# johncai117/Meta-Fine-Tuning

Hardware: AMD Instinct MI355X
Metric: episodes/sec at 5-way N-shot (ResNet10+GNN) per GPU and 1/2/4/8-GPU node (higher is better)
Workload: dtype f32

## Files before the change

### meta-fine-tuning_amd/csrc/conv_igemm.hip

```cpp
#include "mft_common.h"
#include "mft_hip_testing.h"

int mft_stem_conv_dispatch(const float* in, const float* w, float* out, int n_img, int H, int W, int w_ld,
                           hipStream_t s);
int mft_skinny_fwd_dispatch(const float* in, int ldi, const float* w, float* out, int ldo, int n_img, int H, int W,
                            int Cin, int Cout, int KH, int KW, int stride, int pad, int imgs_per_group,
                            long long w_group_stride, hipStream_t s);
void mft_skinny_set_dgrad_slices(int n);
void mft_skinny_set_tap(int v);
void mft_skinny_set_x3(int v);
void mft_skinny_set_nw(int v);
void mft_bn_small_set_rows(int rows);
void mft_bn_fwd_small_set_rows(int rows);
void mft_skinny_set_lines(int v);
int mft_skinny_dgrad_dispatch(const float* dy, int ldy, const float* w, float* dx, int ldx, int n_img, int H, int W,
                              int Cin, int Cout, int KH, int KW, int stride, int pad, int imgs_per_group,
                              long long w_group_stride, hipStream_t s);

namespace {

struct ConvArgs {
    const float* in;
    const float* w;
    const float* bias;
// ... 1197 lines not shown
    else if (tile >= 9100) mft_skinny_set_nw(tile - 9100);
    else if (tile >= 9000) g_wgrad_pol = tile - 9000;
    else if (tile >= 8000) mft_skinny_set_x3(tile - 8000);
    else if (tile >= 7000) mft_skinny_set_tap(tile - 7000);
    else if (tile >= 6000) mft_skinny_set_dgrad_slices(tile - 6000);
    else if (tile >= 5000) g_wgrad_early = tile - 5000;
    else if (tile >= 4000) g_wgrad_min_lds_kb = tile - 4000;
    else if (tile >= 3000) g_skinny = tile - 3000;
    else if (tile >= 2100) g_stem_wgrad_strips = tile - 2100;
    else if (tile >= 2000) g_stem_fast = tile - 2000;
    else if (tile >= 1000) g_wgrad_tile = tile - 1000;
    else g_conv_tile = tile;
    return 0;
}

extern "C" int mft_debug_set_x3_tile(int t);

extern "C" void mft_wgrad_fwd_set_exact(int on);
extern "C" int mft_debug_reset(void) {
    mft_wgrad_fwd_set_exact(0);
    mft_wgrad_fwd_set_xcd(1);
    g_dgrad_parity = 1; g_wgrad_trim = 1; g_wgrad_rows = 1; g_wgrad_tile = 64; g_conv_tile = 0; g_wgrad_pol = 7; g_wgrad_early = 1; g_wgrad_min_lds_kb = 0; g_skinny = 1; g_stem_fast = 1; g_stem_wgrad_strips = 1;
    mft_skinny_set_lines(1); mft_skinny_set_nw(0); mft_skinny_set_x3(1); mft_skinny_set_tap(1); mft_skinny_set_dgrad_slices(1);
    mft_debug_set_x3_tile(0); mft_debug_set_x3_tile(10); mft_debug_set_x3_tile(21); mft_debug_set_x3_tile(31); mft_debug_set_x3_tile(41);
    mft_bn_small_set_rows(512); mft_bn_fwd_small_set_rows(512);
    mft_debug_set_x3_tile(60); mft_debug_set_x3_tile(70); mft_debug_set_x3_tile(80); mft_debug_set_x3_tile(91); mft_debug_set_x3_tile(100); mft_debug_set_x3_tile(200);
    return 0;
}

static int dgrad_impl(const float* dy, int ldy, const float* w, float* dx, int ldx, int n_img, int H,
                      int W, int Cin, int Cout, int KH, int KW, int stride, int pad,
                      int imgs_per_group, long long w_group_stride, float* ws, void* stream) {
    if (Cout % 32 != 0 || Cin % 4 != 0 || ldy % 4 != 0 || stride < 1) return MFT_EINVAL;
    if (imgs_per_group <= 0) imgs_per_group = n_img;
    if (n_img % imgs_per_group != 0) return MFT_EINVAL;
    const int groups = n_img / imgs_per_group;
    if (g_skinny && groups > 1 && w_group_stride != 0 && ws == nullptr) {
        const int rc = mft_skinny_dgrad_dispatch(dy, ldy, w, dx, ldx, n_img, H, W, Cin, Cout, KH, KW, stride, pad,
                                                 imgs_per_group, w_group_stride, (hipStream_t)stream);
        if (rc != MFT_EINVAL) return rc;
    }
    ConvArgs a;
    a.in = dy; a.w = w; a.bias = nullptr; a.out = dx;
    a.ldi = ldy; a.ldo = ldx;
    a.H = (H + 2 * pad - KH) / stride + 1;
    a.W = (W + 2 * pad - KW) / stride + 1;
    a.Cin = Cout; a.KH = KH; a.KW = KW;
// ... 181 lines not shown
```

### meta-fine-tuning_amd/csrc/conv_x3.hip

```cpp
#include "mft_common.h"
#include "bn_fold.h"

namespace {

typedef __bf16 bf16x8 __attribute__((ext_vector_type(8)));
typedef __bf16 bf16x2 __attribute__((ext_vector_type(2)));
typedef _Float16 f16x8 __attribute__((ext_vector_type(8)));
typedef _Float16 f16x4 __attribute__((ext_vector_type(4)));
typedef float f32x2 __attribute__((ext_vector_type(2)));
typedef unsigned u32x2 __attribute__((ext_vector_type(2)));
typedef unsigned u32x4 __attribute__((ext_vector_type(4)));

struct X3Args {
    const float* in;
    const unsigned short* w3;
    long long plane;
    float* out;
    int ldi, ldo;
    int H, W, Cin, OH, OW, Cout, KH, KW, stride, pad;
    int Kpad;
    int M;
    int tiles_n;
    unsigned in_bytes, w_bytes;
    int xcd_swizzle;
// ... 22 lines not shown
    r[0] = x[0] - __builtin_bit_cast(float, p1[0] << 16);
    r[1] = x[1] - __builtin_bit_cast(float, p1[0] & 0xffff0000u);
    r[2] = x[2] - __builtin_bit_cast(float, p1[1] << 16);
    r[3] = x[3] - __builtin_bit_cast(float, p1[1] & 0xffff0000u);
    p2[0] = pk_bf16(r[0], r[1]);
    p2[1] = pk_bf16(r[2], r[3]);
    r[0] -= __builtin_bit_cast(float, p2[0] << 16);
    r[1] -= __builtin_bit_cast(float, p2[0] & 0xffff0000u);
    r[2] -= __builtin_bit_cast(float, p2[1] << 16);
    r[3] -= __builtin_bit_cast(float, p2[1] & 0xffff0000u);
    p3[0] = pk_bf16(r[0], r[1]);
    p3[1] = pk_bf16(r[2], r[3]);
}

__device__ __forceinline__ void split4_h2(const f32x4 x, u32x2& p1, u32x2& p2) {
    const f16x4 hi = __builtin_convertvector(x, f16x4);
    const f32x4 r = (x - __builtin_convertvector(hi, f32x4)) * 2048.f;
    const f16x4 lo = __builtin_convertvector(r, f16x4);
    p1 = __builtin_bit_cast(u32x2, hi);
    p2 = __builtin_bit_cast(u32x2, lo);
}
constexpr float X3_H2_LO_SCALE = 1.0f / 2048.f;

template <int BM, int BN, bool AP, bool DB, int HOIST = 0, int DBG = 0, bool XS = false, int NP = 3>
__global__ __launch_bounds__(256) __attribute__((amdgpu_waves_per_eu(NP == 2 ? 3 : 1))) void conv_x3_kernel(X3Args p) {
    static_assert(NP == 3 || (NP == 2 && !AP && !DB && HOIST == 0 && DBG == 0 && !XS), "f16x2: the plain single-buffer form only");
    constexpr int NACC = NP == 3 ? 1 : 2;
    constexpr int TM = BM / 64;
    constexpr int TN = BN / 64;
    constexpr int PA = AP ? BM / 64 : BM / 32;
    constexpr int PB = BN / 64;
    constexpr int RS = XS ? 32 : X3_RS;
    constexpr int A_PLANE = BM * RS;
    constexpr int B_PLANE = BN * RS;
    auto lo = [](int row, int c) -> int {
        if constexpr (XS) return row * 32 + ((((c >> 3) ^ (row >> 2)) & 3) << 3) + (c & 7);
        else return row * X3_RS + c;
    };
    extern __shared__ __attribute__((aligned(16))) unsigned short smem[];
    unsigned short* As = smem;
    unsigned short* Bs = smem + NP * A_PLANE;
    constexpr int BUF = NP * (A_PLANE + B_PLANE);

    const int tid = threadIdx.x;
    const int lane = tid & 63, wave = tid >> 6;
    const int wm = wave >> 1, wn = wave & 1;
    const int r = lane & 31, h = lane >> 5;
    const bool g_swz = !XS && p.row_swz != 0;
    int tile_id = blockIdx.x;
    if (p.xcd_swizzle) {
        const int nwg = gridDim.x, q = nwg >> 3, rmd = nwg & 7;
        const int xcd = tile_id & 7, slot = tile_id >> 3;
        tile_id = xcd * q + (xcd < rmd ? xcd : rmd) + slot;
    }
    const int nt = tile_id % p.tiles_n;
    const int mt = tile_id / p.tiles_n;
    const int m0 = mt * BM, n0 = nt * BN;

    const int g_id = AP ? tid >> 4 : tid >> 5;
    const int g_rr = AP ? (tid >> 2) & 3 : (tid >> 3) & 3;
    const int lrow = g_swz ? g_rr * 4 + (g_id & 3) + 16 * (g_id >> 2) : (AP ? tid >> 2 : tid >> 3);
    const int c4 = AP ? (tid & 3) * 8 : (tid & 7) * 4;
    constexpr int RPP = AP ? 64 : 32;
    constexpr int ESZ = AP ? 2 : 4;
    const int ohw = p.OH * p.OW;
// ... 1 lines not shown
                                         : __builtin_amdgcn_make_buffer_rsrc((void*)p.in, 0, p.in_bytes, 0x00020000);
    const __amdgpu_buffer_rsrc_t rB = __builtin_amdgcn_make_buffer_rsrc((void*)p.w3, 0, p.w_bytes, 0x00020000);
    int a_off[PA];
    int a_ih0[PA], a_iw0[PA];
    bool a_ok[PA];
#pragma unroll
    for (int j = 0; j < PA; ++j) {
        const int m = m0 + lrow + RPP * j;
        a_ok[j] = m < p.M;
        const int mm = a_ok[j] ? m : 0;
        const int img = mm / ohw;
        const int rem = mm - img * ohw;
        const int oh = rem / p.OW, ow = rem - oh * p.OW;
        a_ih0[j] = oh * p.stride - p.pad;
        a_iw0[j] = ow * p.stride - p.pad;
        a_off[j] = (((img * p.H + a_ih0[j]) * p.W + a_iw0[j]) * p.ldi + c4) * ESZ;
    }
    const int bseg = tid & 3;
    const int brow = g_swz ? ((tid >> 2) & 3) * 4 + ((tid >> 4) & 3) + 16 * (tid >> 6) : tid >> 2;
    int b_off[PB];
#pragma unroll
    for (int j = 0; j < PB; ++j) b_off[j] = ((n0 + brow + 64 * j) * p.Kpad + bseg * 8) * 2;
    const int plane_bytes = (int)(p.plane * 2);

    f32x16 accs[NACC][TM][TN];
#pragma unroll
    for (int q = 0; q < NACC; ++q)
#pragma unroll
        for (int i = 0; i < TM; ++i)
#pragma unroll
            for (int j = 0; j < TN; ++j)
#pragma unroll
                for (int e = 0; e < 16; ++e) accs[q][i][j][e] = 0.f;
    auto& acc = accs[0];
    auto val = [&](int i, int j, int e) -> float {
        if constexpr (NP == 3) return accs[0][i][j][e];
        else return __builtin_fmaf(accs[NACC - 1][i][j][e], X3_H2_LO_SCALE, accs[0][i][j][e]);
    };

    struct Stage {
        f32x4 ra[AP ? 1 : PA];
        u32x4 ra3[AP ? PA : 1][3];
        u32x4 rb[PB][NP];
    };
    Stage st0;
    const int nk = p.Kpad / 32;

    int t_kt = 0, t_ci0 = 0, t_kh = 0, t_kw = 0;
    auto load_tile = [&](int kt, Stage& S) {
        const int k0 = kt * 32;
        while (t_kt < kt) {
            ++t_kt;
            t_ci0 += 32;
            if (t_ci0 == p.Cin) { t_ci0 = 0; if (++t_kw == p.KW) { t_kw = 0; ++t_kh; } }
        }
        const int ci0 = t_ci0, kh = t_kh, kw = t_kw;
        const int tap_off = ((kh * p.W + kw) * p.ldi + ci0) * ESZ;
#pragma unroll
        for (int j = 0; j < PA; ++j) {
            const bool ok = a_ok[j] && (unsigned)(a_ih0[j] + kh) < (unsigned)p.H && (unsigned)(a_iw0[j] + kw) < (unsigned)p.W;
            const unsigned voff = ok ? (unsigned)(a_off[j] + tap_off) : 0x80000000u;
            if constexpr (AP) {
#pragma unroll
                for (int pl = 0; pl < 3; ++pl)
                    S.ra3[j][pl] = __builtin_amdgcn_raw_buffer_load_b128(rA, voff, pl * (int)p.in_plane_bytes, 0);
            } else {
                S.ra[j] = __builtin_bit_cast(f32x4, __builtin_amdgcn_raw_buffer_load_b128(rA, voff, 0, 0));
            }
        }
#pragma unroll
        for (int j = 0; j < PB; ++j)
#pragma unroll
            for (int pl = 0; pl < NP; ++pl)
                S.rb[j][pl] = __builtin_amdgcn_raw_buffer_load_b128(rB, b_off[j] + pl * plane_bytes, k0 * 2, 0);
    };
    auto store_tile = [&](const Stage& S, int buf) {
        unsigned short* As = smem + buf * BUF;
        unsigned short* Bs = As + NP * A_PLANE;
#pragma unroll
        for (int j = 0; j < PA; ++j) {
            const int off = lo(lrow + RPP * j, c4);
            if constexpr (NP == 2) {
                u32x2 p1, p2;
                split4_h2(S.ra[j], p1, p2);
                *(u32x2*)(As + off) = p1;
                *(u32x2*)(As + A_PLANE + off) = p2;
            } else if constexpr (AP) {
#pragma unroll
                for (int pl = 0; pl < 3; ++pl) *(u32x4*)(As + pl * A_PLANE + off) = S.ra3[j][pl];
            } else {
                u32x2 p1, p2, p3;
                if constexpr (DBG & 1) {
                    const u32x4 raw = __builtin_bit_cast(u32x4, S.ra[j]);
                    p1[0] = raw[0]; p1[1] = raw[1]; p2[0] = raw[2]; p2[1] = raw[3]; p3 = p1;
                } else {
                    split4(S.ra[j], p1, p2, p3);
                }
                *(u32x2*)(As + off) = p1;
                *(u32x2*)(As + A_PLANE + off) = p2;
                *(u32x2*)(As + 2 * A_PLANE + off) = p3;
            }
        }
#pragma unroll
        for (int j = 0; j < PB; ++j)
#pragma unroll
            for (int pl = 0; pl < NP; ++pl)
                *(u32x4*)(Bs + pl * B_PLANE + lo(brow + 64 * j, bseg * 8)) = S.rb[j][pl];
    };

    auto compute = [&](int buf) {
        const unsigned short* As = smem + buf * BUF;
        const unsigned short* Bs = As + NP * A_PLANE;
        if constexpr (NP == 2) {
#pragma unroll
            for (int kk = 0; kk < 2; ++kk) {
                f16x8 a[TM][2], b[TN][2];
#pragma unroll
                for (int i = 0; i < TM; ++i)
#pragma unroll
                    for (int pl = 0; pl < 2; ++pl)
                        a[i][pl] = *(const f16x8*)(As + pl * A_PLANE + lo(wm * (BM / 2) + i * 32 + r, kk * 16 + h * 8));
#pragma unroll
                for (int j = 0; j < TN; ++j)
#pragma unroll
                    for (int pl = 0; pl < 2; ++pl)
                        b[j][pl] = *(const f16x8*)(Bs + pl * B_PLANE + lo(wn * (BN / 2) + j * 32 + r, kk * 16 + h * 8));
                constexpr int TA[3] = {0, 1, 0};
                constexpr int TB[3] = {1, 0, 0};
                constexpr int TQ[3] = {1, 1, 0};
#pragma unroll
                for (int t = 0; t < 3; ++t)
#pragma unroll
                    for (int i = 0; i < TM; ++i)
#pragma unroll
                        for (int j = 0; j < TN; ++j)
                            accs[TQ[t] ? NACC - 1 : 0][i][j] =
                                __builtin_amdgcn_mfma_f32_32x32x16_f16(a[i][TA[t]], b[j][TB[t]], accs[TQ[t] ? NACC - 1 : 0][i][j], 0, 0, 0);
            }
            return;
        }
        if constexpr (HOIST == 0) {
#pragma unroll
            for (int kk = 0; kk < 2; ++kk) {
                bf16x8 a[TM][3], b[TN][3];
#pragma unroll
                for (int i = 0; i < TM; ++i)
#pragma unroll
                    for (int pl = 0; pl < 3; ++pl)
                        a[i][pl] = *(const bf16x8*)(As + pl * A_PLANE + lo(wm * (BM / 2) + i * 32 + r, kk * 16 + h * 8));
// ... 79 lines not shown
            rd(1);
            mm(0);
            for (int q = 0; q < 6 * TM * TN; ++q) {
                __builtin_amdgcn_sched_group_barrier(0x8, 1, 0);
                __builtin_amdgcn_sched_group_barrier(0x100, (3 * (TM + TN) + 6 * TM * TN - 1) / (6 * TM * TN), 0);
            }
            __builtin_amdgcn_sched_barrier(0);
            mm(1);
            __builtin_amdgcn_sched_barrier(0);
        }
    };
    if constexpr (DB) {
        load_tile(0, st0);
        store_tile(st0, 0);
        __syncthreads();
        load_tile(nk > 1 ? 1 : 0, st0);
        for (int kt = 0; kt + 1 < nk; ++kt) {
            compute(kt & 1);
            store_tile(st0, (kt + 1) & 1);
            load_tile(kt + 2 < nk ? kt + 2 : nk - 1, st0);
            __syncthreads();
        }
        compute((nk - 1) & 1);
    } else {
        load_tile(0, st0);
        store_tile(st0, 0);
        __syncthreads();
        for (int kt = 0; kt < nk; ++kt) {
            if constexpr (!(DBG & 4)) { if (kt + 1 < nk) load_tile(kt + 1, st0); }
            if constexpr (!(DBG & 16)) compute(0);
            if constexpr (!(DBG & 32)) __syncthreads();
            if constexpr (!(DBG & 8)) { if (kt + 1 < nk) store_tile(st0, 0); }
            if constexpr (!(DBG & 32)) __syncthreads();
        }
    }

#pragma unroll
    for (int i = 0; i < TM; ++i)
#pragma unroll
        for (int j = 0; j < TN; ++j) {
            const int n = n0 + wn * (BN / 2) + j * 32 + r;
#pragma unroll
            for (int e = 0; e < 16; ++e) {
                const int row = (e & 3) + 8 * (e >> 2) + 4 * h;
                const int m = m0 + wm * (BM / 2) + i * 32 + row;
                if (m < p.M) p.out[(long long)m * p.ldo + n] = val(i, j, e);
// ... 25 lines not shown
                o[0] = a1; o[1] = a2; o[2] = b1; o[3] = b2;
            }
        }
        __syncthreads();
        if (wm == 0 && h == 0) {
#pragma unroll
            for (int j = 0; j < TN; ++j) {
                const float* o0 = sred + ((((0 * 2 + wn) * TN + j) * 32 + r) << 2);
                const float* o1 = sred + ((((1 * 2 + wn) * TN + j) * 32 + r) << 2);
                const int n = n0 + wn * (BN / 2) + j * 32 + r;
                float* w0 = p.stats_ws + (((long long)mt * 2 + 0) * p.Cout + n) * 2;
                float* w1 = p.stats_ws + (((long long)mt * 2 + 1) * p.Cout + n) * 2;
                w0[0] = o0[0] + o1[0]; w0[1] = o0[1] + o1[1];
                w1[0] = o0[2] + o1[2]; w1[1] = o0[3] + o1[3];
            }
        }
    }
}

#ifdef MFT_EXPERIMENTS
#include "../../tools/experiments/conv_x3_pingpong.inc"
#endif

template <int BM, int BN, bool BNIN, int NP = 3, bool BDB = true>
__device__ __forceinline__ void conv_x3_s1_body(const X3Args& p) {
    static_assert(NP == 3 || NP == 2, "3 bf16 pieces (six products) or 2 fp16 pieces (three products)");
    constexpr int NACC = NP == 3 ? 1 : 2;
    constexpr int TM = BM / 64, TN = BN / 64;
    constexpr int PA = BM / 32, PB = BN / 64;
    constexpr int RS = X3_RS;
    constexpr int B_PLANE = BN * RS;
    const int A_PLANE = p.s1_rows * RS;
    extern __shared__ __attribute__((aligned(16))) unsigned short smem[];
    constexpr int NBB = (NP == 2 && BDB) ? 2 : 1;
    unsigned short* As = smem;
    unsigned short* Bs = smem + NP * A_PLANE;
    float* bn_tab = reinterpret_cast<float*>(Bs + NBB * NP * B_PLANE);

    const int tid = threadIdx.x;
    const int lane = tid & 63, wave = tid >> 6;
    const int wm = wave >> 1, wn = wave & 1;
    const int r = lane & 31, h = lane >> 5;
    int tile_id = blockIdx.x;
    if (p.xcd_swizzle) {
        const int nwg = gridDim.x, q = nwg >> 3, rmd = nwg & 7;
        const int xcd = tile_id & 7, slot = tile_id >> 3;
        tile_id = xcd * q + (xcd < rmd ? xcd : rmd) + slot;
    }
    const int nt = tile_id % p.tiles_n;
    const int mt = tile_id / p.tiles_n;
    const int m0 = mt * BM, n0 = nt * BN;
    const int W = p.W, H = p.H;
    const int fr0 = m0 / W;
    const int g0 = BNIN ? m0 / p.rows_per_group : 0;
    const bool bn_two = BNIN && (m0 + (BM < p.M - m0 ? BM : p.M - m0) - 1) / p.rows_per_group > g0;
    if constexpr (BNIN) {
        char* stage = reinterpret_cast<char*>(smem);
// ... 26 lines not shown
        const int t = lrow + 32 * j, m = m0 + t;
        const int fr = m / W;
        a_ok[j] = m < p.M;
        a_oh[j] = fr - (fr / H) * H;
        a_off[j] = ((a_ok[j] ? m : 0) * p.ldi + c4) * 4;
        a_lds[j] = (t + 1) * RS + c4;
        a_tab[j] = BNIN ? ((a_ok[j] ? m / p.rows_per_group - g0 : 0) * 2 * p.Cin + c4) : 0;
    }
    const int hside = (tid >> 3) & 1;
    const int mh = hside ? m0 + BM : m0 - 1;
    const int frh = (mh > 0 ? mh : 0) / W;
    const bool h_ok = tid < 16 && (hside ? (mh < p.M && mh - frh * W != 0) : (m0 > 0 && m0 - fr0 * W != 0));
    const int h_oh = frh - (frh / H) * H;
    const int h_off = ((h_ok ? mh : 0) * p.ldi + c4) * 4;
    const int h_lds = (hside ? BM + 1 : 0) * RS + c4;
    const int h_tab = BNIN ? (((hside && h_ok) ? (m0 + BM - 1) / p.rows_per_group - g0 : 0) * 2 * p.Cin + c4) : 0;

    const int bseg = tid & 3;
    const int brow = p.row_swz ? ((tid >> 2) & 3) * 4 + ((tid >> 4) & 3) + 16 * (tid >> 6) : tid >> 2;
    int b_off[PB];
#pragma unroll
    for (int j = 0; j < PB; ++j) b_off[j] = ((n0 + brow + 64 * j) * p.Kpad + bseg * 8) * 2;
    const int plane_bytes = (int)(p.plane * 2);

    int fa[TM], fl[TM], fr_[TM];
    constexpr int Z0 = BM + 2;
#pragma unroll
    for (int i = 0; i < TM; ++i) {
        const int t = wm * (BM / 2) + i * 32 + r;
        const int ow = (m0 + t) - ((m0 + t) / W) * W;
        fa[i] = (t + 1) * RS;
        fl[i] = ow == 0 ? (Z0 + ((t - Z0) & 15)) * RS : fa[i] - RS;
        fr_[i] = ow == W - 1 ? (Z0 + ((t + 2 - Z0) & 15)) * RS : fa[i] + RS;
    }

    f32x16 acc[NACC][TM][TN];
#pragma unroll
    for (int q = 0; q < NACC; ++q)
#pragma unroll
        for (int i = 0; i < TM; ++i)
#pragma unroll
            for (int j = 0; j < TN; ++j)
#pragma unroll
                for (int e = 0; e < 16; ++e) acc[q][i][j][e] = 0.f;
    auto val = [&](int i, int j, int e) -> float {
        if constexpr (NP == 3) return acc[0][i][j][e];
// ... 7 lines not shown
    };
    Stage st;
    const int n_ci = p.Cin / 32;
    const int n_ms = 3 * n_ci;
    auto load_a = [&](int ms, Stage& S) {
        const int kh = ms / n_ci, ci0 = (ms - kh * n_ci) * 32;
        const int shift = ((kh - 1) * W * p.ldi + ci0) * 4;
#pragma unroll
        for (int j = 0; j < PA; ++j) {
            const bool ok = a_ok[j] && (unsigned)(a_oh[j] + kh - 1) < (unsigned)H;
            S.ra[j] = __builtin_bit_cast(f32x4, __builtin_amdgcn_raw_buffer_load_b128(rA, ok ? (unsigned)(a_off[j] + shift) : 0x80000000u, 0, 0));
        }
        const bool okh = h_ok && (unsigned)(h_oh + kh - 1) < (unsigned)H;
        S.rh = __builtin_bit_cast(f32x4, __builtin_amdgcn_raw_buffer_load_b128(rA, okh ? (unsigned)(h_off + shift) : 0x80000000u, 0, 0));
    };
    auto load_b = [&](int ms, int kw, Stage& S) {
        const int kh = ms / n_ci, ci0 = (ms - kh * n_ci) * 32;
        const int k0 = (kh * 3 + kw) * p.Cin + ci0;
#pragma unroll
        for (int j = 0; j < PB; ++j)
#pragma unroll
            for (int pl = 0; pl < NP; ++pl)
                S.rb[j][pl] = __builtin_amdgcn_raw_buffer_load_b128(rB, b_off[j] + pl * plane_bytes, k0 * 2, 0);
    };
    auto put_a = [&](const f32x4 v, int off) {
        if constexpr (NP == 3) {
            u32x2 p1, p2, p3;
            split4(v, p1, p2, p3);
            *(u32x2*)(As + off) = p1;
            *(u32x2*)(As + A_PLANE + off) = p2;
            *(u32x2*)(As + 2 * A_PLANE + off) = p3;
        } else {
            u32x2 p1, p2;
            split4_h2(v, p1, p2);
            *(u32x2*)(As + off) = p1;
            *(u32x2*)(As + A_PLANE + off) = p2;
        }
    };
    auto bn_relu = [&](const f32x4 v, const f32x4 sc, const f32x4 sh, bool ok) {
        f32x4 o = mft_bn_affine4(v, sc, sh);
#pragma unroll
        for (int e = 0; e < 4; ++e) o[e] = ok ? fmaxf(o[e], 0.f) : 0.f;
        return o;
    };
    auto store_a = [&](const Stage& S, int ms) {
        if constexpr (BNIN) {
// ... 42 lines not shown
#pragma unroll
                    for (int pl = 0; pl < 3; ++pl)
                        b[j][pl] = *(const bf16x8*)(Bc + pl * B_PLANE + (wn * (BN / 2) + j * 32 + r) * RS + kk * 16 + h * 8);
                constexpr int TA[6] = {2, 0, 1, 1, 0, 0};
                constexpr int TB[6] = {0, 2, 1, 0, 1, 0};
#pragma unroll
                for (int t = 0; t < 6; ++t)
#pragma unroll
                    for (int i = 0; i < TM; ++i)
#pragma unroll
                        for (int j = 0; j < TN; ++j)
                            acc[0][i][j] = __builtin_amdgcn_mfma_f32_32x32x16_bf16(a[i][TA[t]], b[j][TB[t]], acc[0][i][j], 0, 0, 0);
            } else {
                f16x8 a[TM][2], b[TN][2];
#pragma unroll
                for (int i = 0; i < TM; ++i)
#pragma unroll
                    for (int pl = 0; pl < 2; ++pl)
                        a[i][pl] = *(const f16x8*)(As + pl * A_PLANE + (kw == 0 ? fl[i] : (kw == 1 ? fa[i] : fr_[i])) + kk * 16 + h * 8);
#pragma unroll
                for (int j = 0; j < TN; ++j)
#pragma unroll
                    for (int pl = 0; pl < 2; ++pl)
                        b[j][pl] = *(const f16x8*)(Bc + pl * B_PLANE + (wn * (BN / 2) + j * 32 + r) * RS + kk * 16 + h * 8);
                constexpr int TA[3] = {0, 1, 0};
                constexpr int TB[3] = {1, 0, 0};
                constexpr int TQ[3] = {1, 1, 0};
#pragma unroll
                for (int t = 0; t < 3; ++t)
#pragma unroll
                    for (int i = 0; i < TM; ++i)
#pragma unroll
                        for (int j = 0; j < TN; ++j)
                            acc[TQ[t]][i][j] = __builtin_amdgcn_mfma_f32_32x32x16_f16(a[i][TA[t]], b[j][TB[t]], acc[TQ[t]][i][j], 0, 0, 0);
            }
        }
    };

    for (int i = tid; i < NP * A_PLANE / 8; i += 256) ((u32x4*)As)[i] = (u32x4){0u, 0u, 0u, 0u};
    load_a(0, st);
    load_b(0, 0, st);
    __syncthreads();
    store_a(st, 0);
    store_b(st);
    __syncthreads();
    if constexpr (NBB == 2) {
        int cur = 0;
        for (int ms = 0; ms < n_ms; ++ms) {
            const int msn = ms + 1 < n_ms ? ms + 1 : ms;
            load_b(ms, 1, st);
            compute(0, cur);
            store_b(st, cur ^ 1);
            __syncthreads();
            load_b(ms, 2, st);
            compute(1, cur ^ 1);
            store_b(st, cur);
            __syncthreads();
            load_a(msn, st);
            load_b(msn, 0, st);
            compute(2, cur);
            store_b(st, cur ^ 1);
            __syncthreads();
// ... 3 lines not shown
        }
    } else {
        for (int ms = 0; ms < n_ms; ++ms) {
            const int msn = ms + 1 < n_ms ? ms + 1 : ms;
            load_b(ms, 1, st);
            compute(0);
            __syncthreads();
            store_b(st);
            __syncthreads();
            load_b(ms, 2, st);
            compute(1);
            __syncthreads();
            store_b(st);
            __syncthreads();
            load_a(msn, st);
            load_b(msn, 0, st);
            compute(2);
            __syncthreads();
            store_a(st, msn);
            store_b(st);
            __syncthreads();
        }
    }

#pragma unroll
    for (int i = 0; i < TM; ++i)
#pragma unroll
        for (int j = 0; j < TN; ++j) {
            const int n = n0 + wn * (BN / 2) + j * 32 + r;
#pragma unroll
            for (int e = 0; e < 16; ++e) {
                const int row = (e & 3) + 8 * (e >> 2) + 4 * h;
                const int m = m0 + wm * (BM / 2) + i * 32 + row;
                if (m < p.M) p.out[(long long)m * p.ldo + n] = val(i, j, e);
            }
        }
    if (p.stats_ws != nullptr) {
        static_assert(TN == 1 || TN == 2, "stats epilogue");
        const int split = (m0 / p.rows_per_group + 1) * p.rows_per_group;
        float* sred = reinterpret_cast<float*>(smem);
        __syncthreads();
#pragma unroll
        for (int j = 0; j < TN; ++j) {
            float a1 = 0.f, a2 = 0.f, b1 = 0.f, b2 = 0.f;
#pragma unroll
            for (int i = 0; i < TM; ++i)
// ... 9 lines not shown
            a1 += __shfl_xor(a1, 32, 64); a2 += __shfl_xor(a2, 32, 64);
            b1 += __shfl_xor(b1, 32, 64); b2 += __shfl_xor(b2, 32, 64);
            if (h == 0) {
                float* o = sred + ((((wm * 2 + wn) * TN + j) * 32 + r) << 2);
                o[0] = a1; o[1] = a2; o[2] = b1; o[3] = b2;
            }
        }
        __syncthreads();
        if (wm == 0 && h == 0) {
#pragma unroll
            for (int j = 0; j < TN; ++j) {
                const float* o0 = sred + ((((0 * 2 + wn) * TN + j) * 32 + r) << 2);
                const float* o1 = sred + ((((1 * 2 + wn) * TN + j) * 32 + r) << 2);
                const int n = n0 + wn * (BN / 2) + j * 32 + r;
                float* w0 = p.stats_ws + (((long long)mt * 2 + 0) * p.Cout + n) * 2;
                float* w1 = p.stats_ws + (((long long)mt * 2 + 1) * p.Cout + n) * 2;
                w0[0] = o0[0] + o1[0]; w0[1] = o0[1] + o1[1];
                w1[0] = o0[2] + o1[2]; w1[1] = o0[3] + o1[3];
            }
        }
    }
}

template <int BM, int BN, int NP = 3, bool BDB = true>
__global__ __launch_bounds__(256) __attribute__((amdgpu_waves_per_eu(NP == 2 ? 3 : 1))) void conv_x3_s1_kernel(X3Args p) {
    conv_x3_s1_body<BM, BN, false, NP, BDB>(p);
}

template <int BM, int BN, int NP = 3, bool BDB = true>
__global__ __launch_bounds__(256) __attribute__((amdgpu_waves_per_eu(3, 3))) void conv_x3_s1_bnin_kernel(X3Args p) {
    conv_x3_s1_body<BM, BN, true, NP, BDB>(p);
}

__global__ void x3_stats_finalize_kernel(const float* __restrict__ ws, int C, int M, int R, int BM, float eps,
                                         float* __restrict__ mean, float* __restrict__ rstd) {
    const int c = blockIdx.x * blockDim.x + threadIdx.x;
    const int g = blockIdx.y;
    if (c >= C) return;
    float mu, rs;
    mft_x3_stats_merge(ws, C, c, g, M, R, BM, eps, mu, rs);
    mean[(long long)g * C + c] = mu;
    rstd[(long long)g * C + c] = rs;
}

__global__ __launch_bounds__(256) void split_bf16x3_kernel(const float* __restrict__ w, unsigned short* __restrict__ out,
                                                           long long n) {
    for (long long i = (long long)blockIdx.x * blockDim.x + threadIdx.x; i < n; i += (long long)gridDim.x * blockDim.x) {
        const float x = w[i];
        const unsigned q1 = pk_bf16(x, 0.f) & 0xffffu;
        const float r1 = x - __builtin_bit_cast(float, q1 << 16);
        const unsigned q2 = pk_bf16(r1, 0.f) & 0xffffu;
        const float r2 = r1 - __builtin_bit_cast(float, q2 << 16);
        const unsigned q3 = pk_bf16(r2, 0.f) & 0xffffu;
        out[i] = (unsigned short)q1;
// ... 26 lines not shown
        const float r2 = r1 - __builtin_bit_cast(float, q2 << 16);
        const unsigned q3 = pk_bf16(r2, 0.f) & 0xffffu;
        j.dst[l] = (unsigned short)q1;
        j.dst[j.n + l] = (unsigned short)q2;
        j.dst[2 * j.n + l] = (unsigned short)q3;
    }
}

__global__ __launch_bounds__(256) void split_f16x2_kernel(const float* __restrict__ w, unsigned short* __restrict__ out, long long n) {
    for (long long i = (long long)blockIdx.x * blockDim.x + threadIdx.x; i < n; i += (long long)gridDim.x * blockDim.x) {
        const float x = w[i];
        const _Float16 hi = (_Float16)x;
        const _Float16 lo = (_Float16)((x - (float)hi) * 2048.f);
        out[i] = __builtin_bit_cast(unsigned short, hi);
        out[n + i] = __builtin_bit_cast(unsigned short, lo);
    }
}

int g_x3_db = 0;
int g_x3_dbg = 0;
int g_x3_hoist = 0;
int g_x3_row_swz = 1;
int g_x3_xcd = 1;
int g_x3_min_lds_kb = 0;

template <int BM, int BN, bool AP, bool DB>
int launch_x3(X3Args p, hipStream_t s, int np = 3) {
    const int tiles_m = (p.M + BM - 1) / BM;
    p.tiles_n = p.Cout / BN;
    p.xcd_swizzle = g_x3_xcd;
    p.row_swz = g_x3_row_swz;
    if (np == 2) {
        if constexpr (!AP && !DB) {
            p.row_swz = g_x3_row_swz != 0;
            const size_t lds2 = (size_t)2 * (BM + BN) * X3_RS * sizeof(unsigned short);
            hipLaunchKernelGGL((conv_x3_kernel<BM, BN, false, false, 0, 0, false, 2>), dim3((unsigned)(tiles_m * p.tiles_n)), dim3(256), lds2, s, p);
            return mft_launch_status();
        }
        return MFT_EINVAL;
    }
#ifdef MFT_EXPERIMENTS
    const bool xs = g_x3_row_swz == 2 && !AP && !DB && g_x3_hoist == 0 && g_x3_dbg == 0;
#else
    constexpr bool xs = false;
#endif
    size_t lds = (size_t)(DB ? 2 : 1) * 3 * (BM + BN) * (xs ? 32 : X3_RS) * sizeof(unsigned short);
#ifdef MFT_EXPERIMENTS
    if ((size_t)g_x3_min_lds_kb * 1024 > lds) lds = (size_t)g_x3_min_lds_kb * 1024;
    if (xs) {
        if constexpr (!AP && !DB) {
            hipLaunchKernelGGL((conv_x3_kernel<BM, BN, false, false, 0, 0, true>), dim3((unsigned)(tiles_m * (p.Cout / BN))), dim3(256), lds, s,
                               ([&] { X3Args q = p; q.tiles_n = p.Cout / BN; q.xcd_swizzle = g_x3_xcd; q.row_swz = 0; return q; })());
            return mft_launch_status();
        }
    }
    auto kern = g_x3_hoist == 1 ? conv_x3_kernel<BM, BN, AP, DB, 1> : (g_x3_hoist == 2 ? conv_x3_kernel<BM, BN, AP, DB, 2> : conv_x3_kernel<BM, BN, AP, DB, 0>);
    if (g_x3_dbg && !AP && !DB) {
        switch (g_x3_dbg) {
            case 1: kern = conv_x3_kernel<BM, BN, AP, DB, 0, 1>; break;
// ... 8 lines not shown
            case 34: kern = conv_x3_kernel<BM, BN, AP, DB, 0, 34>; break;
            case 36: kern = conv_x3_kernel<BM, BN, AP, DB, 0, 36>; break;
            case 33: kern = conv_x3_kernel<BM, BN, AP, DB, 0, 33>; break;
            default: break;
        }
    }
#else
    auto kern = conv_x3_kernel<BM, BN, AP, DB, 0>;
#endif
    if (lds > 64 * 1024) {
        hipError_t e = hipFuncSetAttribute((const void*)kern, hipFuncAttributeMaxDynamicSharedMemorySize, 160 * 1024);
        if (e != hipSuccess) return (int)e;
    }
    hipLaunchKernelGGL(kern, dim3((unsigned)(tiles_m * p.tiles_n)), dim3(256), lds, s, p);
    return mft_launch_status();
}

int g_x3_s1 = 1;

constexpr size_t X3_S1_LDS_3PER_CU = 160 * 1024 / 3;

int g_x3_bdb = 1;

inline size_t x3_s1_lds(int BM, int BN, int W, int bn_cin, int np = 3) {
    (void)W;
    return (size_t)np * (BM + 18 + ((np == 2 && g_x3_bdb) ? 2 : 1) * BN) * X3_RS * sizeof(unsigned short) + (size_t)4 * bn_cin * sizeof(float);
}

template <int BM, int BN>
int launch_x3_s1(X3Args p, hipStream_t s, int np = 3) {
    const int tiles_m = (p.M + BM - 1) / BM;
    p.tiles_n = p.Cout / BN;
    p.xcd_swizzle = g_x3_xcd;
    p.row_swz = g_x3_row_swz != 0;
    p.s1_rows = BM + 18;
    const size_t lds = x3_s1_lds(BM, BN, p.W, p.bn_ws ? p.Cin : 0, np);
    const dim3 grid((unsigned)(tiles_m * p.tiles_n));
    if (np == 2 && g_x3_bdb) {
        if (p.bn_ws) hipLaunchKernelGGL((conv_x3_s1_bnin_kernel<BM, BN, 2, true>), grid, dim3(256), lds, s, p);
        else hipLaunchKernelGGL((conv_x3_s1_kernel<BM, BN, 2, true>), grid, dim3(256), lds, s, p);
    } else if (np == 2) {
        if (p.bn_ws) hipLaunchKernelGGL((conv_x3_s1_bnin_kernel<BM, BN, 2, false>), grid, dim3(256), lds, s, p);
        else hipLaunchKernelGGL((conv_x3_s1_kernel<BM, BN, 2, false>), grid, dim3(256), lds, s, p);
    } else if (p.bn_ws) {
        hipLaunchKernelGGL((conv_x3_s1_bnin_kernel<BM, BN>), grid, dim3(256), lds, s, p);
    } else {
        hipLaunchKernelGGL((conv_x3_s1_kernel<BM, BN>), grid, dim3(256), lds, s, p);
    }
    return mft_launch_status();
}

int g_x3_pp = 0;
#ifdef MFT_EXPERIMENTS

template <int BM, int BN>
int launch_x3_pp(X3Args p, hipStream_t s) {
    const int tiles_m = (p.M + BM - 1) / BM;
    p.tiles_n = p.Cout / BN;
    p.xcd_swizzle = g_x3_xcd;
    p.row_swz = 1;
    const size_t lds = (size_t)2 * 3 * (BM + BN) * X3_RS * sizeof(unsigned short);
// ... 25 lines not shown
    return mft_launch_status();
}

extern "C" int mft_split_bf16x3_multi(const void* jobs, int n_jobs, long long total_elements, void* stream) {
    if (n_jobs < 1 || total_elements < 1) return MFT_EINVAL;
    long long blocks = (total_elements + 255) / 256;
    if (blocks > 4096) blocks = 4096;
    hipLaunchKernelGGL(split_bf16x3_multi_kernel, dim3((unsigned)blocks), dim3(256), 0, (hipStream_t)stream, (const SplitJob*)jobs, n_jobs,
                       total_elements);
    return mft_launch_status();
}

extern "C" int mft_debug_set_x3_tile(int t) {
#ifndef MFT_EXPERIMENTS
    const bool off = (t == 10 || t == 60 || t == 70 || t == 80 || t == 100 || t == 200);
    if (!off && ((t >= 10 && t < 20) || t == 42 || (t >= 60 && t < 90) || t >= 100)) return MFT_EINVAL;
#endif
    if (t >= 200) g_x3_dbg = t - 200;
    else if (t >= 100) g_x3_min_lds_kb = t - 100;
    else if (t >= 90) g_x3_s1 = t - 90;
    else if (t >= 80) g_x3_hoist = t - 80;
    else if (t >= 70) g_x3_pp = t - 70;
    else if (t >= 60) g_x3_db = t - 60;
    else if (t >= 40) g_x3_row_swz = t - 40;
    else if (t >= 30) g_x3_bdb = t - 30;
    else if (t >= 20) g_x3_xcd = t - 20;
    else if (t >= 10) g_x3_patch = t - 10;
    else g_x3_tile = t;
    return 0;
}

static int x3_dispatch(const float* in, int ldi, const unsigned short* w3, long long plane_elems, float* out, int ldo,
                       int n_img, int H, int W, int Cin, int Cout, int KH, int KW, int stride, int pad, float* stats_ws,
                       int rows_per_group, void* stream, const unsigned short* in3 = nullptr, long long in_plane_elems = 0,
                       const float* bn_ws = nullptr, const float* bn_gamma = nullptr, const float* bn_beta = nullptr,
                       float bn_eps = 0.f, int np = 3) {
    if (n_img <= 0 || Cin % 32 != 0 || Cout % 64 != 0 || ldi % 4 != 0 || (np != 3 && np != 2)) return MFT_EINVAL;
    if (np == 2 && (in3 != nullptr || g_x3_tile > 1 || g_x3_db || g_x3_pp || g_x3_dbg || g_x3_hoist || g_x3_row_swz == 2 || g_x3_min_lds_kb ||
                    g_x3_patch))
        return MFT_EINVAL;
    X3Args p;
    p.bn_ws = bn_ws; p.bn_gamma = bn_gamma; p.bn_beta = bn_beta; p.bn_eps = bn_eps;
    p.bn_max_tiles = bn_ws ? mft_x3_max_group_tiles(rows_per_group, 128) : 0;
    if (bn_ws != nullptr && (in3 != nullptr || !bn_gamma || !bn_beta || rows_per_group < 128 || KH != 3 || KW != 3 || stride != 1 ||
                             pad != 1 || x3_s1_lds(128, 64, W, Cin, np) > X3_S1_LDS_3PER_CU ||
                             2 * mft_x3_stage_bytes_host(p.bn_max_tiles, Cin) >
// ... 195 lines not shown
```

Measured before the change: 89.22.

## Load x3 conv weight tiles directly into LDS via buffer-load-to-LDS DMA

Adds a path to the f16x2 implicit-GEMM conv kernels that moves 64-column weight tiles straight from global memory into LDS with buffer_load_lds, using a swizzled 32-wide row layout. This removes the register staging and LDS store pass for the B operand. The stride-1 kernel gets a triple-buffered weight pipeline with explicit vmcnt/lgkmcnt barriers, and the general kernel double-buffers B. The path is on by default, changes the LDS sizing, and adds complex hand-written wait logic that can cause hazards or lower occupancy.

```diff
diff --git a/meta-fine-tuning_amd/csrc/conv_igemm.hip b/meta-fine-tuning_amd/csrc/conv_igemm.hip
--- a/meta-fine-tuning_amd/csrc/conv_igemm.hip
+++ b/meta-fine-tuning_amd/csrc/conv_igemm.hip
@@ -1243,7 +1243,7 @@
     mft_wgrad_fwd_set_xcd(1);
     g_dgrad_parity = 1; g_wgrad_trim = 1; g_wgrad_rows = 1; g_wgrad_tile = 64; g_conv_tile = 0; g_wgrad_pol = 7; g_wgrad_early = 1; g_wgrad_min_lds_kb = 0; g_skinny = 1; g_stem_fast = 1; g_stem_wgrad_strips = 1;
     mft_skinny_set_lines(1); mft_skinny_set_nw(0); mft_skinny_set_x3(1); mft_skinny_set_tap(1); mft_skinny_set_dgrad_slices(1);
-    mft_debug_set_x3_tile(0); mft_debug_set_x3_tile(10); mft_debug_set_x3_tile(21); mft_debug_set_x3_tile(31); mft_debug_set_x3_tile(41);
+    mft_debug_set_x3_tile(0); mft_debug_set_x3_tile(10); mft_debug_set_x3_tile(21); mft_debug_set_x3_tile(31); mft_debug_set_x3_tile(41); mft_debug_set_x3_tile(51);
     mft_bn_small_set_rows(512); mft_bn_fwd_small_set_rows(512);
     mft_debug_set_x3_tile(60); mft_debug_set_x3_tile(70); mft_debug_set_x3_tile(80); mft_debug_set_x3_tile(91); mft_debug_set_x3_tile(100); mft_debug_set_x3_tile(200);
     return 0;
diff --git a/meta-fine-tuning_amd/csrc/conv_x3.hip b/meta-fine-tuning_amd/csrc/conv_x3.hip
--- a/meta-fine-tuning_amd/csrc/conv_x3.hip
+++ b/meta-fine-tuning_amd/csrc/conv_x3.hip
@@ -68,9 +68,36 @@
 }
 constexpr float X3_H2_LO_SCALE = 1.0f / 2048.f;
 
-template <int BM, int BN, bool AP, bool DB, int HOIST = 0, int DBG = 0, bool XS = false, int NP = 3>
+typedef __attribute__((address_space(3))) void lds_void_t;
+
+__device__ __forceinline__ int x3_bswz(int row, int c) {
+    return row * 32 + ((((c >> 3) ^ (row >> 2)) & 3) << 3);
+}
+
+__device__ __forceinline__ int x3_bdma_off(int n0, int wave, int lane, int Kpad) {
+    const int row = 16 * wave + (lane >> 2);
+    return ((n0 + row) * Kpad + (((lane & 3) ^ ((row >> 2) & 3)) << 3)) * 2;
+}
+
+template <int NP, int B_PLANE>
+__device__ __forceinline__ void x3_bdma(const __amdgpu_buffer_rsrc_t rB, unsigned short* Bt, int wave_u, int voff, int plane_bytes, int k0) {
+#pragma unroll
+    for (int pl = 0; pl < NP; ++pl)
+        __builtin_amdgcn_raw_ptr_buffer_load_lds(rB, (lds_void_t*)(Bt + pl * B_PLANE + wave_u * 16 * 32), 16, voff + pl * plane_bytes, k0 * 2, 0, 0);
+}
+
+template <int N>
+__device__ __forceinline__ void x3_barrier_vm() {
+    asm volatile("s_waitcnt vmcnt(%0) lgkmcnt(0)\n\ts_barrier" ::"n"(N) : "memory");
+}
+__device__ __forceinline__ void x3_barrier_lds() {
+    asm volatile("s_waitcnt lgkmcnt(0)\n\ts_barrier" ::: "memory");
+}
+
+template <int BM, int BN, bool AP, bool DB, int HOIST = 0, int DBG = 0, bool XS = false, int NP = 3, bool BDMA = false>
 __global__ __launch_bounds__(256) __attribute__((amdgpu_waves_per_eu(NP == 2 ? 3 : 1))) void conv_x3_kernel(X3Args p) {
     static_assert(NP == 3 || (NP == 2 && !AP && !DB && HOIST == 0 && DBG == 0 && !XS), "f16x2: the plain single-buffer form only");
+    static_assert(!BDMA || (NP == 2 && BN == 64), "LDS-DMA weight tiles: f16x2, one 1 KiB piece per wave and plane");
     constexpr int NACC = NP == 3 ? 1 : 2;
     constexpr int TM = BM / 64;
     constexpr int TN = BN / 64;
@@ -78,7 +105,7 @@
     constexpr int PB = BN / 64;
     constexpr int RS = XS ? 32 : X3_RS;
     constexpr int A_PLANE = BM * RS;
-    constexpr int B_PLANE = BN * RS;
+    constexpr int B_PLANE = BN * (BDMA ? 32 : RS);
     auto lo = [](int row, int c) -> int {
         if constexpr (XS) return row * 32 + ((((c >> 3) ^ (row >> 2)) & 3) << 3) + (c & 7);
         else return row * X3_RS + c;
@@ -87,6 +114,10 @@
     unsigned short* As = smem;
     unsigned short* Bs = smem + NP * A_PLANE;
     constexpr int BUF = NP * (A_PLANE + B_PLANE);
+    auto lob = [&](int row, int c) -> int {
+        if constexpr (BDMA) return x3_bswz(row, c);
+        else return lo(row, c);
+    };
 
     const int tid = threadIdx.x;
     const int lane = tid & 63, wave = tid >> 6;
@@ -134,6 +165,8 @@
 #pragma unroll
     for (int j = 0; j < PB; ++j) b_off[j] = ((n0 + brow + 64 * j) * p.Kpad + bseg * 8) * 2;
     const int plane_bytes = (int)(p.plane * 2);
+    const int wave_u = __builtin_amdgcn_readfirstlane(wave);
+    const int d_off = BDMA ? x3_bdma_off(n0, wave, lane, p.Kpad) : 0;
 
     f32x16 accs[NACC][TM][TN];
 #pragma unroll
@@ -159,7 +192,7 @@
     const int nk = p.Kpad / 32;
 
     int t_kt = 0, t_ci0 = 0, t_kh = 0, t_kw = 0;
-    auto load_tile = [&](int kt, Stage& S) {
+    auto load_tile = [&](int kt, Stage& S, int bb = 0) {
         const int k0 = kt * 32;
         while (t_kt < kt) {
             ++t_kt;
@@ -180,11 +213,15 @@
                 S.ra[j] = __builtin_bit_cast(f32x4, __builtin_amdgcn_raw_buffer_load_b128(rA, voff, 0, 0));
             }
         }
-#pragma unroll
-        for (int j = 0; j < PB; ++j)
-#pragma unroll
-            for (int pl = 0; pl < NP; ++pl)
-                S.rb[j][pl] = __builtin_amdgcn_raw_buffer_load_b128(rB, b_off[j] + pl * plane_bytes, k0 * 2, 0);
+        if constexpr (BDMA) {
+            x3_bdma<NP, B_PLANE>(rB, Bs + bb * NP * B_PLANE, wave_u, d_off, plane_bytes, k0);
+        } else {
+#pragma unroll
+            for (int j = 0; j < PB; ++j)
+#pragma unroll
+                for (int pl = 0; pl < NP; ++pl)
+                    S.rb[j][pl] = __builtin_amdgcn_raw_buffer_load_b128(rB, b_off[j] + pl * plane_bytes, k0 * 2, 0);
+        }
     };
     auto store_tile = [&](const Stage& S, int buf) {
         unsigned short* As = smem + buf * BUF;
@@ -213,16 +250,18 @@
                 *(u32x2*)(As + 2 * A_PLANE + off) = p3;
             }
         }
-#pragma unroll
-        for (int j = 0; j < PB; ++j)
-#pragma unroll
-            for (int pl = 0; pl < NP; ++pl)
-                *(u32x4*)(Bs + pl * B_PLANE + lo(brow + 64 * j, bseg * 8)) = S.rb[j][pl];
-    };
-
-    auto compute = [&](int buf) {
+        if constexpr (!BDMA) {
+#pragma unroll
+            for (int j = 0; j < PB; ++j)
+#pragma unroll
+                for (int pl = 0; pl < NP; ++pl)
+                    *(u32x4*)(Bs + pl * B_PLANE + lo(brow + 64 * j, bseg * 8)) = S.rb[j][pl];
+        }
+    };
+
+    auto compute = [&](int buf, int bb = 0) {
         const unsigned short* As = smem + buf * BUF;
-        const unsigned short* Bs = As + NP * A_PLANE;
+        const unsigned short* Bs = As + NP * A_PLANE + bb * NP * B_PLANE;
         if constexpr (NP == 2) {
 #pragma unroll
             for (int kk = 0; kk < 2; ++kk) {
@@ -236,7 +275,7 @@
                 for (int j = 0; j < TN; ++j)
 #pragma unroll
                     for (int pl = 0; pl < 2; ++pl)
-                        b[j][pl] = *(const f16x8*)(Bs + pl * B_PLANE + lo(wn * (BN / 2) + j * 32 + r, kk * 16 + h * 8));
+                        b[j][pl] = *(const f16x8*)(Bs + pl * B_PLANE + lob(wn * (BN / 2) + j * 32 + r, kk * 16 + h * 8));
                 constexpr int TA[3] = {0, 1, 0};
                 constexpr int TB[3] = {1, 0, 0};
                 constexpr int TQ[3] = {1, 1, 0};
@@ -362,6 +401,17 @@
             __syncthreads();
         }
         compute((nk - 1) & 1);
+    } else if constexpr (BDMA) {
+        load_tile(0, st0, 0);
+        store_tile(st0, 0);
+        __syncthreads();
+        for (int kt = 0; kt < nk; ++kt) {
+            if (kt + 1 < nk) load_tile(kt + 1, st0, (kt + 1) & 1);
+            compute(0, kt & 1);
+            x3_barrier_lds();
+            if (kt + 1 < nk) store_tile(st0, 0);
+            x3_barrier_vm<0>();
+        }
     } else {
         load_tile(0, st0);
         store_tile(st0, 0);
@@ -433,17 +483,18 @@
 #include "../../tools/experiments/conv_x3_pingpong.inc"
 #endif
 
-template <int BM, int BN, bool BNIN, int NP = 3, bool BDB = true>
+template <int BM, int BN, bool BNIN, int NP = 3, bool BDB = true, bool BDMA = false>
 __device__ __forceinline__ void conv_x3_s1_body(const X3Args& p) {
     static_assert(NP == 3 || NP == 2, "3 bf16 pieces (six products) or 2 fp16 pieces (three products)");
+    static_assert(!BDMA || (NP == 2 && BDB && BN == 64), "LDS-DMA weight tiles: f16x2 form, one 1 KiB piece per wave and plane");
     constexpr int NACC = NP == 3 ? 1 : 2;
     constexpr int TM = BM / 64, TN = BN / 64;
     constexpr int PA = BM / 32, PB = BN / 64;
     constexpr int RS = X3_RS;
-    constexpr int B_PLANE = BN * RS;
+    constexpr int B_PLANE = BN * (BDMA ? 32 : RS);
     const int A_PLANE = p.s1_rows * RS;
     extern __shared__ __attribute__((aligned(16))) unsigned short smem[];
-    constexpr int NBB = (NP == 2 && BDB) ? 2 : 1;
+    constexpr int NBB = BDMA ? 3 : (NP == 2 && BDB) ? 2 : 1;
     unsigned short* As = smem;
     unsigned short* Bs = smem + NP * A_PLANE;
     float* bn_tab = reinterpret_cast<float*>(Bs + NBB * NP * B_PLANE);
@@ -516,6 +567,8 @@
 #pragma unroll
     for (int j = 0; j < PB; ++j) b_off[j] = ((n0 + brow + 64 * j) * p.Kpad + bseg * 8) * 2;
     const int plane_bytes = (int)(p.plane * 2);
+    const int wave_u = __builtin_amdgcn_readfirstlane(wave);
+    const int d_off = BDMA ? x3_bdma_off(n0, wave, lane, p.Kpad) : 0;
 
     int fa[TM], fl[TM], fr_[TM];
     constexpr int Z0 = BM + 2;
@@ -569,6 +622,10 @@
 #pragma unroll
             for (int pl = 0; pl < NP; ++pl)
                 S.rb[j][pl] = __builtin_amdgcn_raw_buffer_load_b128(rB, b_off[j] + pl * plane_bytes, k0 * 2, 0);
+    };
+    auto dma_b = [&](int ms, int kw, int bb) {
+        const int kh = ms / n_ci, ci0 = (ms - kh * n_ci) * 32;
+        x3_bdma<NP, B_PLANE>(rB, Bs + bb * NP * B_PLANE, wave_u, d_off, plane_bytes, (kh * 3 + kw) * p.Cin + ci0);
     };
     auto put_a = [&](const f32x4 v, int off) {
         if constexpr (NP == 3) {
@@ -657,7 +714,8 @@
                 for (int j = 0; j < TN; ++j)
 #pragma unroll
                     for (int pl = 0; pl < 2; ++pl)
-                        b[j][pl] = *(const f16x8*)(Bc + pl * B_PLANE + (wn * (BN / 2) + j * 32 + r) * RS + kk * 16 + h * 8);
+                        b[j][pl] = *(const f16x8*)(Bc + pl * B_PLANE + (BDMA ? x3_bswz(wn * (BN / 2) + j * 32 + r, kk * 16 + h * 8)
+                                                                              : (wn * (BN / 2) + j * 32 + r) * RS + kk * 16 + h * 8));
                 constexpr int TA[3] = {0, 1, 0};
                 constexpr int TB[3] = {1, 0, 0};
                 constexpr int TQ[3] = {1, 1, 0};
@@ -673,6 +731,31 @@
     };
 
     for (int i = tid; i < NP * A_PLANE / 8; i += 256) ((u32x4*)As)[i] = (u32x4){0u, 0u, 0u, 0u};
+    if constexpr (BDMA) {
+        load_a(0, st);
+        dma_b(0, 0, 0);
+        dma_b(0, 1, 1);
+        __syncthreads();
+        store_a(st, 0);
+        x3_barrier_vm<0>();
+        for (int ms = 0; ms < n_ms; ++ms) {
+            const int msn = ms + 1 < n_ms ? ms + 1 : ms;
+            dma_b(ms, 2, 2);
+            compute(0, 0);
+            x3_barrier_vm<NP>();
+            dma_b(msn, 0, 0);
+            compute(1, 1);
+            x3_barrier_vm<NP>();
+            load_a(msn, st);
+            __builtin_amdgcn_sched_barrier(0);
+            dma_b(msn, 1, 1);
+            compute(2, 2);
+            x3_barrier_lds();
+            store_a(st, msn);
+            x3_barrier_vm<NP>();
+        }
+        x3_barrier_vm<0>();
+    } else {
     load_a(0, st);
     load_b(0, 0, st);
     __syncthreads();
@@ -722,6 +805,7 @@
             __syncthreads();
         }
     }
+    }
 
 #pragma unroll
     for (int i = 0; i < TM; ++i)
@@ -777,14 +861,14 @@
     }
 }
 
-template <int BM, int BN, int NP = 3, bool BDB = true>
+template <int BM, int BN, int NP = 3, bool BDB = true, bool BDMA = false>
 __global__ __launch_bounds__(256) __attribute__((amdgpu_waves_per_eu(NP == 2 ? 3 : 1))) void conv_x3_s1_kernel(X3Args p) {
-    conv_x3_s1_body<BM, BN, false, NP, BDB>(p);
-}
-
-template <int BM, int BN, int NP = 3, bool BDB = true>
+    conv_x3_s1_body<BM, BN, false, NP, BDB, BDMA>(p);
+}
+
+template <int BM, int BN, int NP = 3, bool BDB = true, bool BDMA = false>
 __global__ __launch_bounds__(256) __attribute__((amdgpu_waves_per_eu(3, 3))) void conv_x3_s1_bnin_kernel(X3Args p) {
-    conv_x3_s1_body<BM, BN, true, NP, BDB>(p);
+    conv_x3_s1_body<BM, BN, true, NP, BDB, BDMA>(p);
 }
 
 __global__ void x3_stats_finalize_kernel(const float* __restrict__ ws, int C, int M, int R, int BM, float eps,
@@ -857,6 +941,7 @@
 int g_x3_hoist = 0;
 int g_x3_row_swz = 1;
 int g_x3_xcd = 1;
+int g_x3_dma = 1;
 int g_x3_min_lds_kb = 0;
 
 template <int BM, int BN, bool AP, bool DB>
@@ -868,8 +953,14 @@
     if (np == 2) {
         if constexpr (!AP && !DB) {
             p.row_swz = g_x3_row_swz != 0;
-            const size_t lds2 = (size_t)2 * (BM + BN) * X3_RS * sizeof(unsigned short);
-            hipLaunchKernelGGL((conv_x3_kernel<BM, BN, false, false, 0, 0, false, 2>), dim3((unsigned)(tiles_m * p.tiles_n)), dim3(256), lds2, s, p);
+            const dim3 grid((unsigned)(tiles_m * p.tiles_n));
+            if (g_x3_dma && BN == 64) {
+                const size_t lds2 = (size_t)2 * (BM * X3_RS + 2 * BN * 32) * sizeof(unsigned short);
+                hipLaunchKernelGGL((conv_x3_kernel<BM, BN, false, false, 0, 0, false, 2, BN == 64>), grid, dim3(256), lds2, s, p);
+            } else {
+                const size_t lds2 = (size_t)2 * (BM + BN) * X3_RS * sizeof(unsigned short);
+                hipLaunchKernelGGL((conv_x3_kernel<BM, BN, false, false, 0, 0, false, 2>), grid, dim3(256), lds2, s, p);
+            }
             return mft_launch_status();
         }
         return MFT_EINVAL;
@@ -924,9 +1015,12 @@
 
 int g_x3_bdb = 1;
 
+inline bool x3_s1_dma(int np) { return np == 2 && g_x3_bdb && g_x3_dma; }
+
 inline size_t x3_s1_lds(int BM, int BN, int W, int bn_cin, int np = 3) {
     (void)W;
-    return (size_t)np * (BM + 18 + ((np == 2 && g_x3_bdb) ? 2 : 1) * BN) * X3_RS * sizeof(unsigned short) + (size_t)4 * bn_cin * sizeof(float);
+    const size_t b_elems = x3_s1_dma(np) ? (size_t)3 * BN * 32 : (size_t)((np == 2 && g_x3_bdb) ? 2 : 1) * BN * X3_RS;
+    return ((size_t)np * (BM + 18) * X3_RS + np * b_elems) * sizeof(unsigned short) + (size_t)4 * bn_cin * sizeof(float);
 }
 
 template <int BM, int BN>
@@ -938,7 +1032,10 @@
     p.s1_rows = BM + 18;
     const size_t lds = x3_s1_lds(BM, BN, p.W, p.bn_ws ? p.Cin : 0, np);
     const dim3 grid((unsigned)(tiles_m * p.tiles_n));
-    if (np == 2 && g_x3_bdb) {
+    if (x3_s1_dma(np) && BN == 64) {
+        if (p.bn_ws) hipLaunchKernelGGL((conv_x3_s1_bnin_kernel<BM, BN, 2, true, BN == 64>), grid, dim3(256), lds, s, p);
+        else hipLaunchKernelGGL((conv_x3_s1_kernel<BM, BN, 2, true, BN == 64>), grid, dim3(256), lds, s, p);
+    } else if (np == 2 && g_x3_bdb) {
         if (p.bn_ws) hipLaunchKernelGGL((conv_x3_s1_bnin_kernel<BM, BN, 2, true>), grid, dim3(256), lds, s, p);
         else hipLaunchKernelGGL((conv_x3_s1_kernel<BM, BN, 2, true>), grid, dim3(256), lds, s, p);
     } else if (np == 2) {
@@ -1010,6 +1107,7 @@
     else if (t >= 80) g_x3_hoist = t - 80;
     else if (t >= 70) g_x3_pp = t - 70;
     else if (t >= 60) g_x3_db = t - 60;
+    else if (t >= 50) { if (t > 51) return MFT_EINVAL; g_x3_dma = t - 50; }
     else if (t >= 40) g_x3_row_swz = t - 40;
     else if (t >= 30) g_x3_bdb = t - 30;
     else if (t >= 20) g_x3_xcd = t - 20;
```

After: 89.82, median of 6. No clear change (+0.7%).
